# rehakvoj1/BIH-GPU-Raytracer

Hardware: NVIDIA B200
Metric: Mrays/s (higher is better)
Workload: dtype f32

## Files before the change

bih-gpu-raytracer_b200/csrc/trace.cu:

```cuda
#include "bihrt_internal.cuh"
#include <float.h>

#define FULL 0xffffffffu
#define NONE 0xFFFFFFFFu
#define TRACE_THREADS 128
#define TRACE_MIN_BLOCKS 8
constexpr int NODE_STEPS = 4;

#define OCT_MIXED 8
#define BOX_EPS 2.384185791015625e-07f

#define DET_EPS __uint_as_float(0x358637beu)

struct Hit { float t; int slot; };

__device__ __forceinline__ float fmin3(float a, float b, float c) { float r; asm("min.f32 %0, %1, %2, %3;" : "=f"(r) : "f"(a), "f"(b), "f"(c)); return r; }
__device__ __forceinline__ float fmax3(float a, float b, float c) { float r; asm("max.f32 %0, %1, %2, %3;" : "=f"(r) : "f"(a), "f"(b), "f"(c)); return r; }

__device__ __forceinline__ uint32_t pack_colour(uint32_t hits, int samples) {
    const float fh = (float)hits, fm = (float)(samples - (int)hits), fs = (float)samples;
    float cr = __fdiv_rn(__fadd_rn(__fmul_rn(fh, 255.f), __fmul_rn(fm, 20.f)), fs);
    float cb = __fdiv_rn(__fmul_rn(fm, 40.f), fs);
    cr = fmaxf(0.f, fminf(255.f, cr));
    cb = fmaxf(0.f, fminf(255.f, cb));
    return ((uint32_t)(int)cb << 16) | ((uint32_t)(int)cr << 8) | (uint32_t)(int)cr;
}

__device__ __forceinline__ float mt_det(float dx, float dy, float dz, float e1x, float e1y, float e1z, float e2x, float e2y, float e2z,
                                        float& px, float& py, float& pz) {
    px = __fsub_rn(__fmul_rn(dy, e2z), __fmul_rn(e2y, dz));
    py = __fsub_rn(__fmul_rn(dz, e2x), __fmul_rn(e2z, dx));
    pz = __fsub_rn(__fmul_rn(dx, e2y), __fmul_rn(e2x, dy));
    return __fadd_rn(__fadd_rn(__fmul_rn(e1x, px), __fmul_rn(e1y, py)), __fmul_rn(e1z, pz));
}
__device__ __forceinline__ float mt_u(float ox, float oy, float oz, const float4& q0, float px, float py, float pz, float inv,
                                      float& tx, float& ty, float& tz) {
    tx = __fsub_rn(ox, q0.x); ty = __fsub_rn(oy, q0.y); tz = __fsub_rn(oz, q0.z);
    return __fmul_rn(__fadd_rn(__fadd_rn(__fmul_rn(tx, px), __fmul_rn(ty, py)), __fmul_rn(tz, pz)), inv);
}
__device__ __forceinline__ float mt_v(float dx, float dy, float dz, float e1x, float e1y, float e1z, float tx, float ty, float tz, float inv,
                                      float& qx, float& qy, float& qz) {
    qx = __fsub_rn(__fmul_rn(ty, e1z), __fmul_rn(e1y, tz));
    qy = __fsub_rn(__fmul_rn(tz, e1x), __fmul_rn(e1z, tx));
    qz = __fsub_rn(__fmul_rn(tx, e1y), __fmul_rn(e1x, ty));
    return __fmul_rn(__fadd_rn(__fadd_rn(__fmul_rn(dx, qx), __fmul_rn(dy, qy)), __fmul_rn(dz, qz)), inv);
}

template <bool COUNTED, bool FIRST, bool RANGE = false, bool TWO_SIDED = false>
__device__ __forceinline__ void test_leaf(const char* __restrict__ first_tri, float ox, float oy, float oz,
                                          float dx, float dy, float dz, Hit& h, uint32_t& ntris, uint32_t& wleaf,
                                          const float* tlo_p = nullptr) {
    const float4* p = reinterpret_cast<const float4*>(first_tri);
    for (;;) {
        const float4 q0 = __ldg(p), q1 = __ldg(p + 1), q2 = __ldg(p + 2);
        if (COUNTED) { ntris++; const uint32_t am = __activemask(); wleaf += ((threadIdx.x & 31) == __ffs(am) - 1); }
        const float e1x = q0.w, e1y = q1.x, e1z = q1.y, e2x = q1.z, e2y = q1.w, e2z = q2.x;
        float px, py, pz;
        const float det = mt_det(dx, dy, dz, e1x, e1y, e1z, e2x, e2y, e2z, px, py, pz);
        if (!((TWO_SIDED ? fabsf(det) : det) < DET_EPS)) {
            const float inv = __frcp_rn(det);
            float tx, ty, tz;
            const float u = mt_u(ox, oy, oz, q0, px, py, pz, inv, tx, ty, tz);
            if (!(u < 0.f || u > 1.f)) {
                float qx, qy, qz;
                const float v = mt_v(dx, dy, dz, e1x, e1y, e1z, tx, ty, tz, inv, qx, qy, qz);
                if (!(v < 0.f || __fadd_rn(u, v) > 1.f)) {
                    const float t = __fmul_rn(__fadd_rn(__fadd_rn(__fmul_rn(e2x, qx), __fmul_rn(e2y, qy)), __fmul_rn(e2z, qz)), inv);
                    if (t > (RANGE ? *tlo_p : 0.f) && t < h.t) {
                        h.t = t; h.slot = (int)__float_as_uint(q2.w);
                        if (FIRST) break;
                    }
                }
            }
        }
        if (__float_as_uint(q2.z) & 1u) break;
        p += 3;
    }
}

template <int MODE, bool COUNTED, bool Q>
__global__ void __launch_bounds__(TRACE_THREADS, TRACE_MIN_BLOCKS) k_trace(TraceArgs a) {
    constexpr int STACK_DEPTH = Q ? STACK_DEPTH_QUALITY : STACK_DEPTH_PARITY;
    constexpr bool COVER = MODE == 1;
    constexpr bool OCTS = MODE == 1;
    constexpr bool LIST = MODE == 0 || MODE == 3 || MODE == 4;
    constexpr bool RANGE = MODE == 3 || MODE == 4;
    constexpr bool TWO_SIDED = MODE == 4;
    __shared__ __align__(16) float s_ray[TRACE_THREADS * 10];
    const int lane = threadIdx.x & 31;
    const uint32_t lt = (1u << lane) - 1u;
    float* my_ray = s_ray + threadIdx.x * 10;
    const char* __restrict__ nodes_b = reinterpret_cast<const char*>(a.nodes);
    const char* __restrict__ tris_b = reinterpret_cast<const char*>(a.tris);
    const BihTri* __restrict__ tris = a.tris;
    const uint32_t nu = a.hdr->nu;
    if (a.hdr->status != 0) return;
    if ((a.hdr->quality != 0) != Q) {
        if (blockIdx.x == 0 && threadIdx.x == 0 && a.status_map) *a.status_map = 0x100u;
        return;
    }
    const float blo[3] = { a.hdr->lo[0], a.hdr->lo[1], a.hdr->lo[2] }, bhi[3] = { a.hdr->hi[0], a.hdr->hi[1], a.hdr->hi[2] };
    uint32_t nnodes = 0, ntris = 0, maxsp = 0;
    uint32_t wnode = 0, wleaf = 0;

    uint64_t total;
    int tx = 1;
    if (LIST) total = a.tile_cost ? (((uint64_t)a.nrays + 1023u) >> 10) << 10 : (uint64_t)a.nrays;
    else {
        tx = (a.w + 31) / 32;
        const int ty = (a.h + 31) / 32, T = tx * ty;
        const int my_tiles = T > a.shard_index ? (T - a.shard_index + a.shard_count - 1) / a.shard_count : 0;
        total = ((uint64_t)my_tiles * 1024u) << a.gshift;
    }
    const int gshift = LIST ? 0 : a.gshift;
    const int nsamp = LIST ? 1 : ((a.s_end - a.s_begin) >> gshift);
    uint32_t my_queue = 0;
    if (a.queues > 1) { asm("mov.u32 %0, %%smid;" : "=r"(my_queue)); my_queue %= (uint32_t)a.queues; }
    uint64_t pool_next = 0, pool_end = 0;
    long long unit_t0 = 0; uint32_t unit_tile = 0xFFFFFFFFu;
    bool exhausted = false;

    uint64_t item = ~0ull;
    int s = 0, s0 = 0;
    uint32_t hits = 0, pixel = 0, pxy = 0;
    float ix = 1.f, iy = 1.f, iz = 1.f, nx = 0.f, ny = 0.f, nz = 0.f, bpad = 0.f;
    uint32_t cur = NONE;
    float rMin = 0.f, pMin = 0.f, pMax = 0.f;
    Hit h; h.t = FLT_MAX; h.slot = -1;
    bool tracing = false;
    uint4 stack[STACK_DEPTH];
    int sp = 0;
#define STACK_RESET() do { sp = 0; } while (0)
#define STACK_PUSH(item) do { stack[sp] = (item); sp++; } while (0)
#define STACK_POP(e) do { sp--; (e) = stack[sp]; } while (0)
    const uint32_t root_ref = BIH_REF_NODE(0, a.hdr->root_axis);
    const bool direct = MODE == 1 && gshift > 0 && !(a.flags & BIHRT_RENDER_COUNTS);
    const uint32_t ray_smem = (uint32_t)__cvta_generic_to_shared(my_ray);

    for (;;) {
        const uint32_t busy = ~__ballot_sync(FULL, cur == NONE);
        if (busy == 0) {
            bool want_item = false, finishing = false;
            if (cur == NONE) {
                if (tracing) {
                    tracing = false;
                    if (MODE == 1) hits += (h.slot >= 0);
                    else if (RANGE) {
                        const bool hit = h.slot >= 0;
                        const bool rec = a.out_u || a.out_v || a.out_ng;
                        float u = 0.f, v = 0.f, gx = 0.f, gy = 0.f, gz = 0.f;
                        int32_t prim = -1;
                        if (hit && (rec || a.out_prim)) {
                            const float4* tq = reinterpret_cast<const float4*>(tris + h.slot);
                            const float4 q0 = __ldg(tq), q1 = __ldg(tq + 1), q2 = __ldg(tq + 2);
                            prim = (int32_t)__float_as_uint(q2.y);
                            if (rec) {
                                const float e1x = q0.w, e1y = q1.x, e1z = q1.y, e2x = q1.z, e2y = q1.w, e2z = q2.x;
                                const float2 dxy = *reinterpret_cast<const float2*>(my_ray + 6);
                                const float dx = dxy.x, dy = dxy.y, dz = my_ray[8];
                                float px, py, pz, tx, ty, tz, qx, qy, qz;
                                const float inv = __frcp_rn(mt_det(dx, dy, dz, e1x, e1y, e1z, e2x, e2y, e2z, px, py, pz));
                                u = mt_u(my_ray[0], my_ray[2], my_ray[4], q0, px, py, pz, inv, tx, ty, tz);
                                v = mt_v(dx, dy, dz, e1x, e1y, e1z, tx, ty, tz, inv, qx, qy, qz);
                                gx = __fsub_rn(__fmul_rn(e1y, e2z), __fmul_rn(e1z, e2y));
                                gy = __fsub_rn(__fmul_rn(e1z, e2x), __fmul_rn(e1x, e2z));
                                gz = __fsub_rn(__fmul_rn(e1x, e2y), __fmul_rn(e1y, e2x));
                            }
                        }
                        if (a.out_t) a.out_t[item] = hit ? h.t : FLT_MAX;
                        if (a.out_slot) a.out_slot[item] = h.slot;
                        if (a.out_prim) a.out_prim[item] = prim;
                        if (a.out_u) a.out_u[item] = u;
                        if (a.out_v) a.out_v[item] = v;
                        if (a.out_ng) { float* g = a.out_ng + 3 * item; g[0] = gx; g[1] = gy; g[2] = gz; }
                    } else {
                        const uint64_t o = MODE == 0 ? item : (uint64_t)pixel * (uint32_t)a.spp + (uint32_t)(s0 + s);
                        if (a.out_t) a.out_t[o] = h.t;
                        if (a.out_slot) a.out_slot[o] = h.slot;
                        if (a.out_prim) a.out_prim[o] = h.slot >= 0 ? (int32_t)tris[h.slot].prim : -1;
                    }
                    s++;
                    if (s == nsamp) {
                        if (MODE == 1 && gshift > 0) finishing = true;
                        else if (MODE == 1 && (a.flags & BIHRT_RENDER_COUNTS)) a.fb[pixel] = hits;
                        else if (MODE == 1) a.fb[pixel] = pack_colour(hits, nsamp);
                        item = ~0ull;
                    }
                }
                want_item = (item == ~0ull);
            }
            if (MODE == 1 && gshift > 0) {
                const uint32_t fin = __ballot_sync(FULL, finishing);
                if (finishing) {
                    const uint32_t same = __match_any_sync(fin, pixel);
                    const uint32_t sum = __reduce_add_sync(same, hits);
                    if (lane == __ffs(same) - 1) {
                        if (direct) a.fb[pixel] = pack_colour(sum, nsamp << gshift);
                        else if (sum) atomicAdd(&a.fb[pixel], sum);
                    }
                }
            }
            if (!LIST && a.tile_cost && unit_tile != 0xFFFFFFFFu) {
                if (lane == 0) atomicMax(a.tile_cost + unit_tile, (uint32_t)min((unsigned long long)(clock64() - unit_t0) >> 8, 0xFFFFFFFFull));
                unit_tile = 0xFFFFFFFFu;
            }
            uint32_t want = __ballot_sync(FULL, want_item);
            while (want && !exhausted) {
                if (pool_next >= pool_end) {
                    uint64_t base = ~0ull;
                    uint32_t got = 0;
                    if (lane == 0) {
                        const uint32_t ilc = (uint32_t)a.il_count, ili = (uint32_t)a.il_index, ics = (uint32_t)a.il_cshift;
                        if (a.queues <= 1) {
                            const uint64_t fetched = atomicAdd(a.work, 32u); got = 32;
                            const uint64_t lu = fetched >> 5;
                            base = ilc > 1 ? ((((lu >> ics) * ilc + ili) << ics) | (lu & ((1u << ics) - 1u))) << 5 : fetched;
                            if (base >= total) base = ~0ull;
                        } else {
                            const uint32_t tshift = 10 + gshift, ushift = 5 + gshift;
                            const uint64_t ntile = (total + ((1ull << tshift) - 1)) >> tshift;
                            for (uint32_t k = 0; k < (uint32_t)a.queues; k++) {
                                uint32_t q = my_queue + k; if (q >= (uint32_t)a.queues) q -= (uint32_t)a.queues;
                                if (q >= ntile) continue;
                                const uint32_t upt = (1u << ushift) / ilc;
                                const uint64_t units = ((ntile - q + a.queues - 1) / a.queues) * upt;
                                if (ld_relaxed(a.work + q) >= units) continue;
                                const uint32_t u = atomicAdd(a.work + q, 1u);
                                if (u >= units) continue;
                                const uint32_t lu = u % upt;
                                const uint64_t b = (((uint64_t)(u / upt) * a.queues + q) << tshift) + ((uint64_t)((((lu >> ics) * ilc + ili) << ics) | (lu & ((1u << ics) - 1u))) << 5);
                                if (b < total) { base = b; got = 32; break; }
                            }
                        }
                    }
                    base = __shfl_sync(FULL, base, 0);
                    got = __shfl_sync(FULL, got, 0);
                    if (LIST && a.tile_cost && unit_tile != 0xFFFFFFFFu) {
                        if (lane == 0) atomicMax(a.tile_cost + unit_tile, (uint32_t)min((unsigned long long)(clock64() - unit_t0) >> 8, 0xFFFFFFFFull));
                        unit_tile = 0xFFFFFFFFu;
                    }
                    if (base == ~0ull) { exhausted = true; break; }
                    pool_next = base;
                    pool_end = min(base + got, total);
                    if (a.tile_cost && unit_tile == 0xFFFFFFFFu) {
                        const uint32_t m = (uint32_t)(base >> (10 + gshift));
                        unit_tile = a.tile_order ? __ldg(a.tile_order + m) : m;
                        unit_t0 = clock64();
                    }
                }
                const uint64_t avail = pool_end - pool_next;
                const uint32_t rank = __popc(want & lt);
                const bool served = want_item && (uint64_t)rank < avail;
                if (served) {
                    item = pool_next + rank; s = 0; hits = 0; want_item = false;
                    if (LIST && a.tile_cost) {
                        const uint32_t mi = (uint32_t)(item >> 10);
                        const uint64_t ray = ((uint64_t)(a.tile_order ? __ldg(a.tile_order + mi) : mi) << 10) | (item & 1023u);
                        item = ray < (uint64_t)a.nrays ? ray : ~0ull;
                        if (item == ~0ull) want_item = true;
                    }
                    if (MODE == 0 && a.perm && item != ~0ull) item = __ldg(a.perm + item);
                    if (!LIST) {
                        const uint64_t pix = item >> gshift;
                        s0 = a.s_begin + (int)((uint32_t)item & ((1u << gshift) - 1u)) * nsamp;
                        const uint32_t mi = (uint32_t)(pix >> 10), q = (uint32_t)pix & 1023u;
                        const uint32_t m = a.tile_order ? __ldg(a.tile_order + mi) : mi;
                        const int tile = a.shard_index + (int)m * a.shard_count;
                        const int px = (tile % tx) * 32 + (int)((q >> 5) & 3u) * 8 + (int)(q & 7u);
                        const int py = (tile / tx) * 32 + (int)(q >> 7) * 4 + (int)((q >> 3) & 3u);
                        if (px < a.w && py < a.h) { pixel = (uint32_t)(py * a.w + px); pxy = (uint32_t)px | ((uint32_t)py << 16); }
                        else item = ~0ull;
                        if (item == ~0ull) want_item = true;
                    }
                }
                pool_next += min((uint64_t)__popc(want), avail);
                want = __ballot_sync(FULL, want_item);
            }
            if (cur == NONE && item != ~0ull) {
                float ox, oy, oz, dx, dy, dz;
                float tlo = 0.f, thi = FLT_MAX;
                bool live = true;
                if (RANGE) {
                    const float4* p = reinterpret_cast<const float4*>(a.rays_iv + item);
                    const float4 r0 = __ldg(p), r1 = __ldg(p + 1);
                    ox = r0.x; oy = r0.y; oz = r0.z; dx = r1.x; dy = r1.y; dz = r1.z;
                    tlo = fmaxf(r0.w, 0.f);
                    live = r0.w == r0.w && tlo < r1.w;
                    thi = fminf(r1.w, FLT_MAX);
                } else if (MODE == 0) {
                    const float* p = reinterpret_cast<const float*>(a.rays + item);
                    ox = __ldg(p); oy = __ldg(p + 1); oz = __ldg(p + 2); dx = __ldg(p + 3); dy = __ldg(p + 4); dz = __ldg(p + 5);
                } else {
                    const int px = (int)(pxy & 0xFFFFu), py = (int)(pxy >> 16);
                    const float ru = (a.flags & BIHRT_RENDER_JITTER) ? bihrt_jitter(a.seed, pixel, (uint32_t)(s0 + s), 0) : 0.5f;
                    const float rv = (a.flags & BIHRT_RENDER_JITTER) ? bihrt_jitter(a.seed, pixel, (uint32_t)(s0 + s), 1) : 0.5f;
                    const float uu = __fdiv_rn(__fadd_rn((float)px, ru), (float)a.w);
                    const float vv = __fdiv_rn(__fadd_rn((float)py, rv), (float)a.h);
                    ox = a.cam.origin[0]; oy = a.cam.origin[1]; oz = a.cam.origin[2];
                    dx = __fsub_rn(__fadd_rn(__fadd_rn(a.cam.lower_left[0], __fmul_rn(uu, a.cam.horizontal[0])), __fmul_rn(vv, a.cam.vertical[0])), ox);
                    dy = __fsub_rn(__fadd_rn(__fadd_rn(a.cam.lower_left[1], __fmul_rn(uu, a.cam.horizontal[1])), __fmul_rn(vv, a.cam.vertical[1])), oy);
                    dz = __fsub_rn(__fadd_rn(__fadd_rn(a.cam.lower_left[2], __fmul_rn(uu, a.cam.horizontal[2])), __fmul_rn(vv, a.cam.vertical[2])), oz);
                }
                ix = __frcp_rn(dx); iy = __frcp_rn(dy); iz = __frcp_rn(dz);
                nx = -__fmul_rn(ox, ix); ny = -__fmul_rn(oy, iy); nz = -__fmul_rn(oz, iz);
                bpad = __fmul_rn(BOX_EPS, fmaxf(fmaxf(fabsf(nx) <= FLT_MAX ? fabsf(nx) : 0.f, fabsf(ny) <= FLT_MAX ? fabsf(ny) : 0.f),
                                                fabsf(nz) <= FLT_MAX ? fabsf(nz) : 0.f));
                *reinterpret_cast<float2*>(my_ray) = make_float2(ox, ix); *reinterpret_cast<float2*>(my_ray + 2) = make_float2(oy, iy);
                *reinterpret_cast<float2*>(my_ray + 4) = make_float2(oz, iz); *reinterpret_cast<float2*>(my_ray + 6) = make_float2(dx, dy);
                my_ray[8] = dz;
                if (RANGE) my_ray[9] = tlo;
                h.t = RANGE ? thi : (MODE == 0 && a.any_hit) ? a.tmax : FLT_MAX; h.slot = -1; STACK_RESET(); tracing = true;
                bool in = nu > 0 && live;
                float tMin = __fmul_rn(__fsub_rn(ix < 0.f ? bhi[0] : blo[0], ox), ix);
                float tMax = __fmul_rn(__fsub_rn(ix < 0.f ? blo[0] : bhi[0], ox), ix);
                const float tymin = __fmul_rn(__fsub_rn(iy < 0.f ? bhi[1] : blo[1], oy), iy);
                const float tymax = __fmul_rn(__fsub_rn(iy < 0.f ? blo[1] : bhi[1], oy), iy);
                if ((tMin > tymax) || (tymin > tMax)) in = false;
                if (tymin > tMin) tMin = tymin;
                if (tymax < tMax) tMax = tymax;
                const float tzmin = __fmul_rn(__fsub_rn(iz < 0.f ? bhi[2] : blo[2], oz), iz);
                const float tzmax = __fmul_rn(__fsub_rn(iz < 0.f ? blo[2] : bhi[2], oz), iz);
                if ((tMin > tzmax) || (tzmin > tMax)) in = false;
                if (tzmin > tMin) tMin = tzmin;
                if (tzmax < tMax) tMax = tzmax;
                if (in) {
                    const float tabs = fmaxf(fabsf(tMin), fabsf(tMax));
                    bpad = __fmaf_rn(BOX_EPS, tabs <= FLT_MAX ? tabs : FLT_MAX, bpad);
                    const float qnan = __uint_as_float(0x7fc00000u);
                    ix = fabsf(ix) <= FLT_MAX ? ix : qnan; iy = fabsf(iy) <= FLT_MAX ? iy : qnan; iz = fabsf(iz) <= FLT_MAX ? iz : qnan;
                    rMin = tMin; pMin = fmaxf(tMin, tlo); pMax = ((MODE == 0 && a.any_hit) || COVER || RANGE) ? fminf(tMax, h.t) : tMax;
                    if (nu == 1) { cur = BIH_REF_LEAFREF(0); pMin = -FLT_MAX; pMax = FLT_MAX; }
                    else if (pMin <= pMax) cur = root_ref;
                }
            }
            if (OCTS) {
                int oct = OCT_MIXED;
                if (gshift > 0) {
                    const bool w = cur != NONE;
                    const uint32_t xn = __ballot_sync(FULL, w && ix < 0.f), xp = __ballot_sync(FULL, w && ix > 0.f);
                    const uint32_t yn = __ballot_sync(FULL, w && iy < 0.f), yp = __ballot_sync(FULL, w && iy > 0.f);
                    const uint32_t zn = __ballot_sync(FULL, w && iz < 0.f), zp = __ballot_sync(FULL, w && iz > 0.f);
                    if (!((xn && xp) || (yn && yp) || (zn && zp))) oct = (xn != 0) | (yn != 0) << 1 | (zn != 0) << 2;
                }
                my_ray[9] = __int_as_float(oct);
            }
            if (__ballot_sync(FULL, cur != NONE || tracing) == 0 && exhausted &&
                __ballot_sync(FULL, item != ~0ull) == 0) break;
        }

#define BOX_SLAB(lx, ly, lz, hx, hy, hz, bn, bf)                                                            \
        do {                                                                                                \
            const float ax0 = __fmaf_rn((lx), ix, nx), ax1 = __fmaf_rn((hx), ix, nx);                       \
            const float ay0 = __fmaf_rn((ly), iy, ny), ay1 = __fmaf_rn((hy), iy, ny);                       \
            const float az0 = __fmaf_rn((lz), iz, nz), az1 = __fmaf_rn((hz), iz, nz);                       \
            float n_, f_;                                                                                   \
            if (OCT == OCT_MIXED) {                                                                         \
                n_ = fmaxf(fmaxf(fminf(ax0, ax1), fminf(ay0, ay1)), fminf(az0, az1));                       \
                f_ = fminf(fminf(fmaxf(ax0, ax1), fmaxf(ay0, ay1)), fmaxf(az0, az1));                       \
            } else {                                             \
                n_ = fmax3((OCT & 1) ? ax1 : ax0, (OCT & 2) ? ay1 : ay0, (OCT & 4) ? az1 : az0);            \
                f_ = fmin3((OCT & 1) ? ax0 : ax1, (OCT & 2) ? ay0 : ay1, (OCT & 4) ? az0 : az1);            \
            }                                                                                               \
            (bn) = __fsub_rn(n_, bpad);                                                                     \
            (bf) = __fadd_rn(f_, bpad);                                                                     \
        } while (0)
#define POP_VALID()                                                                                         \
        do {                                                                                                \
            cur = NONE;                                                                                     \
            if (COVER) {                                   \
                if (sp > 0) {                                                                               \
                    uint4 e;                                                                                \
                    STACK_POP(e);                                                                           \
                    cur = e.x; rMin = __uint_as_float(e.y); pMin = __uint_as_float(e.z); pMax = __uint_as_float(e.w); \
                }                                                                                           \
            } else while (sp > 0) {                                                                         \
                uint4 e;                                                                                    \
                STACK_POP(e);                                                                               \
                const float m = fminf(__uint_as_float(e.w), h.t);                                           \
                if (__uint_as_float(e.z) <= m) { cur = e.x; rMin = __uint_as_float(e.y); pMin = __uint_as_float(e.z); pMax = m; break; } \
            }                                                                                               \
        } while (0)
#ifdef BIHRT_DEBUG_STACK
#define DEBUG_STACK_TRAP() do { if (sp >= STACK_DEPTH) __trap(); } while (0)
#else
#define DEBUG_STACK_TRAP() do { } while (0)
#endif
#define NODE_PHASE(OCT_)                                                                                           \
        do {                                                                                                        \
            constexpr int OCT = (OCT_);                                                                             \
            for (;;) {                                                                                              \
                _Pragma("unroll (NODE_STEPS)")                                                                      \
                for (int rep = 0; rep < NODE_STEPS && (int)cur >= 0; rep++) {                                       \
                                    \
                    float2 oi;                                                                                      \
                    uint32_t ra;                                                                                    \
                    asm("mad.lo.u32 %0, %1, 8, %2;" : "=r"(ra) : "r"(cur & 3u), "r"(ray_smem));                     \
                    asm volatile("ld.shared.v2.f32 {%0, %1}, [%2];" : "=f"(oi.x), "=f"(oi.y) : "r"(ra));            \
                           \
                    const float4* np;                                                                               \
                    asm("mad.wide.u32 %0, %1, 64, %2;" : "=l"(np) : "r"(cur >> 2), "l"(nodes_b));                   \
                     \
                     \
                     \
                     \
                     \
                                                                          \
                    float4 nd, b0, b1, b2;                                                                          \
                    if (LIST) {                                                                                     \
                        asm("ld.global.nc.v8.f32 {%0,%1,%2,%3,%4,%5,%6,%7}, [%8];"                                  \
                            : "=f"(nd.x), "=f"(nd.y), "=f"(nd.z), "=f"(nd.w), "=f"(b0.x), "=f"(b0.y), "=f"(b0.z), "=f"(b0.w) : "l"(np)); \
                        asm("ld.global.nc.v8.f32 {%0,%1,%2,%3,%4,%5,%6,%7}, [%8];"                                  \
                            : "=f"(b1.x), "=f"(b1.y), "=f"(b1.z), "=f"(b1.w), "=f"(b2.x), "=f"(b2.y), "=f"(b2.z), "=f"(b2.w) : "l"(np + 2)); \
                    } else { nd = __ldg(np); b0 = __ldg(np + 1); b1 = __ldg(np + 2); b2 = __ldg(np + 3); }          \
                    if (COUNTED) { nnodes++; const uint32_t am = __activemask(); wnode += (lane == __ffs(am) - 1); } \
                    const uint32_t rl = __float_as_uint(nd.z), rr = __float_as_uint(nd.w);                          \
                    const bool neg = oi.y < 0.f;                                       \
                    const float t0 = __fmul_rn(__fsub_rn(nd.x, oi.x), oi.y);                          \
                    const float t1 = __fmul_rn(__fsub_rn(nd.y, oi.x), oi.y);                                        \
                    const float tn = neg ? t1 : t0, tf = neg ? t0 : t1;                                             \
                    const uint32_t refn = neg ? rr : rl, reff = neg ? rl : rr;                                      \
                     \
                     \
                     \
                     \
                                                              \
                    float bnL, bfL, bnR, bfR;                                                                       \
                    BOX_SLAB(b0.x, b0.y, b0.z, b0.w, b1.x, b1.y, bnL, bfL);                                         \
                    BOX_SLAB(b1.z, b1.w, b2.x, b2.y, b2.z, b2.w, bnR, bfR);                                         \
                     \
                    const float nLo = fmaxf(pMin, neg ? bnR : bnL), nHi = fmin3(pMax, tn, neg ? bfR : bfL);         \
                    const float fLo = fmax3(pMin, tf, neg ? bnL : bnR), fHi = fminf(pMax, neg ? bfL : bfR);         \
                    const bool go_near = (Q || rMin < tn) && (nLo <= nHi);    \
                    const bool go_far = (fLo <= fHi);                                                               \
                     \
                          \
                    if (go_near && go_far) {                                                                        \
                             \
                        if ((int)refn >= 0 && (int)reff < 0) {                                                      \
                            STACK_PUSH(make_uint4(refn, __float_as_uint(rMin), __float_as_uint(nLo), __float_as_uint(nHi))); \
                            cur = reff; rMin = tf; pMin = fLo; pMax = fHi;                                          \
                        } else {                                                                                    \
                            STACK_PUSH(make_uint4(reff, __float_as_uint(tf), __float_as_uint(fLo), __float_as_uint(fHi))); \
                            cur = refn; pMin = nLo; pMax = nHi;                                                     \
                        }                                                                                           \
                         \
                         \
                                                           \
                        if (COUNTED) { maxsp = max(maxsp, (uint32_t)sp); if (sp >= STACK_DEPTH) { maxsp = 0x7fffffffu; sp = STACK_DEPTH - 1; } } \
                        DEBUG_STACK_TRAP();                                                                         \
                    } else if (go_near) { cur = refn; pMin = nLo; pMax = nHi; }                                     \
                    else if (go_far) { cur = reff; rMin = tf; pMin = fLo; pMax = fHi; }                             \
                    else POP_VALID();                                                                               \
                }                                                                                                   \
                const uint32_t m_walk = __ballot_sync(FULL, (int)cur >= 0);                                         \
                if (m_walk == 0) break;                                                                             \
                const uint32_t m_wait = __ballot_sync(FULL, cur + 1u > 0x80000000u);   \
                if (__popc(m_wait) > __popc(m_walk)) break;                                                         \
            }                                                                                                       \
        } while (0)
        if constexpr (!OCTS) NODE_PHASE(OCT_MIXED);
        else switch (__float_as_int(my_ray[9])) {
            case 0: NODE_PHASE(0); break;
            case 1: NODE_PHASE(1); break;
            case 2: NODE_PHASE(2); break;
            case 3: NODE_PHASE(3); break;
            case 4: NODE_PHASE(4); break;
            case 5: NODE_PHASE(5); break;
            case 6: NODE_PHASE(6); break;
            case 7: NODE_PHASE(7); break;
            default: NODE_PHASE(OCT_MIXED); break;
        }
        if (cur + 1u > 0x80000000u) {
            const char* tp;
            asm("mad.wide.u32 %0, %1, 12, %2;" : "=l"(tp) : "r"(cur & 0x7FFFFFFCu), "l"(tris_b));
            const float2 dxy = *reinterpret_cast<const float2*>(my_ray + 6);
            test_leaf<COUNTED, COVER, RANGE, TWO_SIDED>(tp, my_ray[0], my_ray[2], my_ray[4], dxy.x, dxy.y, my_ray[8], h, ntris, wleaf, my_ray + 9);
            if (((LIST && a.any_hit) || COVER) && h.slot >= 0) { STACK_RESET(); cur = NONE; }
            else POP_VALID();
        }
#undef NODE_PHASE
#undef DEBUG_STACK_TRAP
#undef POP_VALID
#undef BOX_SLAB
#undef STACK_RESET
#undef STACK_PUSH
#undef STACK_POP
        __syncwarp();
    }

    if (COUNTED) {
#pragma unroll
        for (int o = 16; o > 0; o >>= 1) {
            nnodes += __shfl_xor_sync(FULL, nnodes, o);
            ntris += __shfl_xor_sync(FULL, ntris, o);
            maxsp = max(maxsp, __shfl_xor_sync(FULL, maxsp, o));
        }
        if (lane == 0) {
            atomicAdd(&a.counters[0], (unsigned long long)nnodes);
            atomicAdd(&a.counters[1], (unsigned long long)ntris);
            atomicMax(&a.counters[2], (unsigned long long)maxsp);
        }
        wnode = __reduce_add_sync(FULL, wnode); wleaf = __reduce_add_sync(FULL, wleaf);
        if (lane == 0) { atomicAdd(&a.counters[4], (unsigned long long)wnode); atomicAdd(&a.counters[5], (unsigned long long)wleaf); }
    }
}

__global__ void k_resolve(uint32_t* fb, int npix, int spp) {
    const int i = blockIdx.x * blockDim.x + threadIdx.x;
    if (i >= npix) return;
    fb[i] = pack_colour(fb[i], spp);
}

#define TILE_CLASSES 5
__device__ __forceinline__ int tile_class(uint32_t c, uint32_t mx) {
    int k = 0;
#pragma unroll
    for (int j = 1; j < TILE_CLASSES; j++) k += c < max(1u, mx >> j);
    return k;
}
__global__ void __launch_bounds__(1024) k_tile_order(uint32_t* __restrict__ cost, uint32_t* __restrict__ order, uint32_t ntiles) {
    __shared__ uint32_t s_w[TILE_CLASSES][32];
    __shared__ uint32_t s_max, s_base[TILE_CLASSES];
    const int lane = threadIdx.x & 31, w = threadIdx.x >> 5;
    const uint32_t per = (ntiles + 1023u) / 1024u, i0 = min(ntiles, threadIdx.x * per), i1 = min(ntiles, i0 + per);
    uint32_t mx = 0;
    for (uint32_t i = i0; i < i1; i++) mx = max(mx, cost[i]);
    mx = __reduce_max_sync(0xffffffffu, mx);
    if (lane == 0) s_w[0][w] = mx;
    __syncthreads();
    if (threadIdx.x == 0) { uint32_t m = 0; for (int k = 0; k < 32; k++) m = max(m, s_w[0][k]); s_max = m; }
    __syncthreads();
    mx = s_max;
    uint32_t cnt[TILE_CLASSES], inc[TILE_CLASSES];
#pragma unroll
    for (int k = 0; k < TILE_CLASSES; k++) cnt[k] = 0;
    for (uint32_t i = i0; i < i1; i++) {
        const int cl = tile_class(cost[i], mx);
#pragma unroll
        for (int k = 0; k < TILE_CLASSES; k++) cnt[k] += (cl == k);
    }
    __syncthreads();
#pragma unroll
    for (int k = 0; k < TILE_CLASSES; k++) {
        inc[k] = cnt[k];
#pragma unroll
        for (int o = 1; o < 32; o <<= 1) { const uint32_t t = __shfl_up_sync(0xffffffffu, inc[k], o); if (lane >= o) inc[k] += t; }
        if (lane == 31) s_w[k][w] = inc[k];
    }
    __syncthreads();
    if (threadIdx.x < TILE_CLASSES) {
        uint32_t run = 0;
        for (int j = 0; j < 32; j++) { const uint32_t x = s_w[threadIdx.x][j]; s_w[threadIdx.x][j] = run; run += x; }
        s_base[threadIdx.x] = run;
    }
    __syncthreads();
    if (threadIdx.x == 0) { uint32_t run = 0; for (int k = 0; k < TILE_CLASSES; k++) { const uint32_t x = s_base[k]; s_base[k] = run; run += x; } }
    __syncthreads();
    uint32_t pos[TILE_CLASSES];
#pragma unroll
    for (int k = 0; k < TILE_CLASSES; k++) pos[k] = s_base[k] + s_w[k][w] + inc[k] - cnt[k];
    for (uint32_t i = i0; i < i1; i++) {
        const int cl = tile_class(cost[i], mx);
#pragma unroll
        for (int k = 0; k < TILE_CLASSES; k++) if (cl == k) order[pos[k]++] = i;
    }
    __syncthreads();
    for (uint32_t i = i0; i < i1; i++) cost[i] = 0;
}

__global__ void __launch_bounds__(1024) k_tile_sort(uint32_t* __restrict__ cost, uint32_t* __restrict__ order, uint32_t ntiles) {
    __shared__ uint32_t s_cnt[256], s_off[256];
    if (threadIdx.x < 256) s_cnt[threadIdx.x] = 0;
    __syncthreads();
    for (uint32_t i = threadIdx.x; i < ntiles; i += 1024) atomicAdd(&s_cnt[min(255u, cost[i] >> 4)], 1u);
    __syncthreads();
    if (threadIdx.x == 0) { uint32_t run = 0; for (int b = 255; b >= 0; b--) { s_off[b] = run; run += s_cnt[b]; } }
    __syncthreads();
    for (uint32_t i = threadIdx.x; i < ntiles; i += 1024) order[atomicAdd(&s_off[min(255u, cost[i] >> 4)], 1u)] = i;
    __syncthreads();
    for (uint32_t i = threadIdx.x; i < ntiles; i += 1024) cost[i] = 0;
}

int bihrt_tile_order_launch(bihrt_ctx* c, uint32_t* cost, uint32_t* order, uint32_t ntiles, bool full_sort) {
    if (full_sort) k_tile_sort<<<1, 1024, 0, c->stream>>>(cost, order, ntiles);
    else k_tile_order<<<1, 1024, 0, c->stream>>>(cost, order, ntiles);
    c->kernel_launches += 1;
    BIHRT_CUDA(c, cudaGetLastError());
    return BIHRT_OK;
}

int bihrt_resolve_launch(bihrt_ctx* c, uint32_t* fb, int npix, int spp) {
    k_resolve<<<(npix + 255) / 256, 256, 0, c->stream>>>(fb, npix, spp);
    c->kernel_launches += 1;
    BIHRT_CUDA(c, cudaGetLastError());
    return BIHRT_OK;
}

template <int MODE, bool COUNTED, bool Q>
static int launch(bihrt_ctx* c, const TraceArgs& a) {
    int per_sm = c->opt_trace_blocks_per_sm;
    if (per_sm <= 0) {
        BIHRT_CUDA(c, cudaOccupancyMaxActiveBlocksPerMultiprocessor(&per_sm, k_trace<MODE, COUNTED, Q>, TRACE_THREADS, 0));
        if (per_sm < 1) per_sm = 1;
    }
    BIHRT_CUDA(c, cudaMemsetAsync(a.work, 0, 4 * 1024, c->stream));
    k_trace<MODE, COUNTED, Q><<<c->sm_count * per_sm, TRACE_THREADS, 0, c->stream>>>(a);
    c->kernel_launches += 1;
    BIHRT_CUDA(c, cudaGetLastError());
    return BIHRT_OK;
}

template <bool Q>
static int launch_mode(bihrt_ctx* c, const TraceArgs& a, int mode, bool counted) {
    switch (mode * 2 + (counted ? 1 : 0)) {
        case 0: return launch<0, false, Q>(c, a);
        case 1: return launch<0, true, Q>(c, a);
        case 2: return launch<1, false, Q>(c, a);
        case 3: return launch<1, true, Q>(c, a);
        case 4: return launch<2, false, Q>(c, a);
        case 5: return launch<2, true, Q>(c, a);
        case 6: return launch<3, false, Q>(c, a);
        case 8: return launch<4, false, Q>(c, a);
        default: return bihrt_fail(c, BIHRT_ERR_INVALID, "bad trace mode %d", mode);
    }
}

int bihrt_trace_launch(bihrt_ctx* c, const TraceArgs& a_in, int mode, bool counted) {
    TraceArgs a = a_in;
    const bool list = mode == 0 || mode == 3 || mode == 4;
    const int64_t rays = list ? a.nrays : (int64_t)a.w * a.h * (a.s_end - a.s_begin) / (a.shard_count > 0 ? a.shard_count : 1) / (a.il_count > 0 ? a.il_count : 1);
    const bool on = a.queues < 0 ? (rays >= (16ll << 20) && (list || a.gshift == 0)) : a.queues != 0;
    a.queues = on ? (c->sm_count < 1024 ? c->sm_count : 1024) : 1;
    uint32_t ntiles = 0;
    bihrt_ctx::TileKey key;
    if (!list) {
        const int tx = (a.w + 31) / 32, ty = (a.h + 31) / 32, T = tx * ty;
        const int mine = T > a.shard_index ? (T - a.shard_index + a.shard_count - 1) / a.shard_count : 0;
        if ((((uint64_t)mine * 1024u) << a.gshift) >= (1ull << 32) - (1ull << 24))
            return bihrt_fail(c, BIHRT_ERR_INVALID, "launch of %d tiles x 1024 pixels x %d lane groups exceeds the 32-bit work counter", mine, 1 << a.gshift);
    }
    const bool order_on = a.queues == 1 && (c->opt_tile_order > 1 || (c->opt_tile_order == 1 && rays >= (64ll << 10) && rays < (48ll << 20) && c->n >= 10000));
    if (order_on) {
        if (list) {
            if (a.nrays > 1024 && a.nrays <= (65536ll << 10)) { ntiles = (uint32_t)((a.nrays + 1023) >> 10); key.nrays = a.nrays; }
        } else {
            const int tx = (a.w + 31) / 32, ty = (a.h + 31) / 32, T = tx * ty;
            const int mine = T > a.shard_index ? (T - a.shard_index + a.shard_count - 1) / a.shard_count : 0;
            if (mine > 1 && mine <= 65536) ntiles = (uint32_t)mine;
            key.w = a.w; key.h = a.h; key.gshift = a.gshift; key.nsamp = a.s_end - a.s_begin; key.shard_index = a.shard_index;
            key.shard_count = a.shard_count; key.il_index = a.il_index; key.il_count = a.il_count; key.il_cshift = a.il_cshift;
        }
        key.mode = list ? mode : 1; key.ntiles = ntiles;
    }
    bihrt_ctx::TileSlot* slot = nullptr;
    if (ntiles) {
        for (auto& ts : c->tile_slots) if (ts.cap && ts.key == key) slot = &ts;
        if (!slot) {
            slot = &c->tile_slots[c->tile_next];
            c->tile_next = (c->tile_next + 1) % 4;
            slot->key = key; slot->valid = false;
        }
        if ((size_t)ntiles > slot->cap) {
            if (slot->cost) cudaFree(slot->cost);
            if (slot->order) cudaFree(slot->order);
            slot->cost = slot->order = nullptr; slot->cap = 0; slot->valid = false;
            if (cudaMalloc(&slot->cost, (size_t)ntiles * 4) != cudaSuccess || cudaMalloc(&slot->order, (size_t)ntiles * 4) != cudaSuccess) {
                cudaGetLastError();
                if (slot->cost) { cudaFree(slot->cost); slot->cost = nullptr; }
                slot = nullptr; ntiles = 0;
            } else slot->cap = ntiles;
        }
        if (slot) {
            if (!slot->valid) BIHRT_CUDA(c, cudaMemsetAsync(slot->cost, 0, (size_t)ntiles * 4, c->stream));
            a.tile_cost = slot->cost;
            a.tile_order = slot->valid ? slot->order : nullptr;
        }
    }
    a.status_map = c->d_status_map;
    int rc = c->built_quality ? launch_mode<true>(c, a, mode, counted) : launch_mode<false>(c, a, mode, counted);
    if (rc == BIHRT_OK && slot) {
        if ((rc = bihrt_tile_order_launch(c, slot->cost, slot->order, ntiles, rays < c->opt_tile_sort_below)) == BIHRT_OK) slot->valid = true;
    }
    return rc;
}
```

Baseline: 14690.

## Pack ray slab math into f32x2 ops and spill per-lane state to shared memory

Rewrites the box-slab and split-plane tests to use paired f32x2 FMA/add/mul instructions on packed 64-bit ray constants. Moves rarely used per-lane scalars (pixel, pxy, s0, unit timestamp) into shared memory, narrows the work-pool counters to 32-bit, and loads the scene bounds only at ray setup. The aim is fewer FP instructions and lower register pressure in the traversal loop, which may allow better occupancy. The costs are extra pack/unpack moves and shared-memory traffic for the moved state, and 32-bit counters that overflow if the work total is very large.

```diff
diff --git a/bih-gpu-raytracer_b200/csrc/trace.cu b/bih-gpu-raytracer_b200/csrc/trace.cu
--- a/bih-gpu-raytracer_b200/csrc/trace.cu
+++ b/bih-gpu-raytracer_b200/csrc/trace.cu
@@ -16,6 +16,18 @@
 
 __device__ __forceinline__ float fmin3(float a, float b, float c) { float r; asm("min.f32 %0, %1, %2, %3;" : "=f"(r) : "f"(a), "f"(b), "f"(c)); return r; }
 __device__ __forceinline__ float fmax3(float a, float b, float c) { float r; asm("max.f32 %0, %1, %2, %3;" : "=f"(r) : "f"(a), "f"(b), "f"(c)); return r; }
+
+__device__ __forceinline__ uint64_t f2_hold(float x, float y) { uint64_t r; asm volatile("mov.b64 %0, {%1, %2};" : "=l"(r) : "f"(x), "f"(y)); return r; }
+__device__ __forceinline__ float f2_x(uint64_t p) { float x, y; asm("mov.b64 {%0, %1}, %2;" : "=f"(x), "=f"(y) : "l"(p)); return x; }
+__device__ __forceinline__ float f2_y(uint64_t p) { float x, y; asm("mov.b64 {%0, %1}, %2;" : "=f"(x), "=f"(y) : "l"(p)); return y; }
+__device__ __forceinline__ float2 f2_fma(float2 a, uint64_t b, uint64_t c) {
+    uint64_t r; asm("{ .reg .b64 t; mov.b64 t, {%1, %2}; fma.rn.f32x2 %0, t, %3, %4; }" : "=l"(r) : "f"(a.x), "f"(a.y), "l"(b), "l"(c));
+    return make_float2(f2_x(r), f2_y(r));
+}
+__device__ __forceinline__ float2 f2_add(float2 a, uint64_t b) {
+    uint64_t r; asm("{ .reg .b64 t; mov.b64 t, {%1, %2}; add.rn.f32x2 %0, t, %3; }" : "=l"(r) : "f"(a.x), "f"(a.y), "l"(b));
+    return make_float2(f2_x(r), f2_y(r));
+}
 
 __device__ __forceinline__ uint32_t pack_colour(uint32_t hits, int samples) {
     const float fh = (float)hits, fm = (float)(samples - (int)hits), fs = (float)samples;
@@ -99,31 +111,36 @@
         if (blockIdx.x == 0 && threadIdx.x == 0 && a.status_map) *a.status_map = 0x100u;
         return;
     }
-    const float blo[3] = { a.hdr->lo[0], a.hdr->lo[1], a.hdr->lo[2] }, bhi[3] = { a.hdr->hi[0], a.hdr->hi[1], a.hdr->hi[2] };
     uint32_t nnodes = 0, ntris = 0, maxsp = 0;
     uint32_t wnode = 0, wleaf = 0;
 
-    uint64_t total;
+    uint32_t total;
     int tx = 1;
-    if (LIST) total = a.tile_cost ? (((uint64_t)a.nrays + 1023u) >> 10) << 10 : (uint64_t)a.nrays;
+    if (LIST) total = (uint32_t)(a.tile_cost ? (((uint64_t)a.nrays + 1023u) >> 10) << 10 : (uint64_t)a.nrays);
     else {
         tx = (a.w + 31) / 32;
         const int ty = (a.h + 31) / 32, T = tx * ty;
         const int my_tiles = T > a.shard_index ? (T - a.shard_index + a.shard_count - 1) / a.shard_count : 0;
-        total = ((uint64_t)my_tiles * 1024u) << a.gshift;
+        total = (uint32_t)(((uint64_t)my_tiles * 1024u) << a.gshift);
     }
     const int gshift = LIST ? 0 : a.gshift;
     const int nsamp = LIST ? 1 : ((a.s_end - a.s_begin) >> gshift);
     uint32_t my_queue = 0;
     if (a.queues > 1) { asm("mov.u32 %0, %%smid;" : "=r"(my_queue)); my_queue %= (uint32_t)a.queues; }
-    uint64_t pool_next = 0, pool_end = 0;
-    long long unit_t0 = 0; uint32_t unit_tile = 0xFFFFFFFFu;
+    uint32_t pool_next = 0, pool_end = 0;
+    uint32_t unit_tile = 0xFFFFFFFFu;
+    __shared__ long long s_unit_t0[TRACE_THREADS / 32];
+    long long& unit_t0 = s_unit_t0[threadIdx.x >> 5];
     bool exhausted = false;
 
     uint64_t item = ~0ull;
-    int s = 0, s0 = 0;
-    uint32_t hits = 0, pixel = 0, pxy = 0;
-    float ix = 1.f, iy = 1.f, iz = 1.f, nx = 0.f, ny = 0.f, nz = 0.f, bpad = 0.f;
+    int s = 0;
+    uint32_t hits = 0;
+    __shared__ uint32_t s_lane[3][TRACE_THREADS];
+    int& s0 = *reinterpret_cast<int*>(&s_lane[0][threadIdx.x]);
+    uint32_t& pixel = s_lane[1][threadIdx.x]; uint32_t& pxy = s_lane[2][threadIdx.x];
+    s0 = 0; pixel = 0; pxy = 0;
+    uint64_t i_xy = f2_hold(1.f, 1.f), i_zx = i_xy, n_xy = f2_hold(0.f, 0.f), n_zx = n_xy, pad = n_xy;
     uint32_t cur = NONE;
     float rMin = 0.f, pMin = 0.f, pMax = 0.f;
     Hit h; h.t = FLT_MAX; h.slot = -1;
@@ -200,8 +217,8 @@
                     }
                 }
             }
-            if (!LIST && a.tile_cost && unit_tile != 0xFFFFFFFFu) {
-                if (lane == 0) atomicMax(a.tile_cost + unit_tile, (uint32_t)min((unsigned long long)(clock64() - unit_t0) >> 8, 0xFFFFFFFFull));
+            if (!LIST && a.tile_cost && lane == 0 && unit_tile != 0xFFFFFFFFu) {
+                atomicMax(a.tile_cost + unit_tile, (uint32_t)min((unsigned long long)(clock64() - unit_t0) >> 8, 0xFFFFFFFFull));
                 unit_tile = 0xFFFFFFFFu;
             }
             uint32_t want = __ballot_sync(FULL, want_item);
@@ -233,24 +250,24 @@
                             }
                         }
                     }
-                    base = __shfl_sync(FULL, base, 0);
+                    const uint32_t first = __shfl_sync(FULL, (uint32_t)base, 0);
                     got = __shfl_sync(FULL, got, 0);
-                    if (LIST && a.tile_cost && unit_tile != 0xFFFFFFFFu) {
-                        if (lane == 0) atomicMax(a.tile_cost + unit_tile, (uint32_t)min((unsigned long long)(clock64() - unit_t0) >> 8, 0xFFFFFFFFull));
+                    if (LIST && a.tile_cost && lane == 0 && unit_tile != 0xFFFFFFFFu) {
+                        atomicMax(a.tile_cost + unit_tile, (uint32_t)min((unsigned long long)(clock64() - unit_t0) >> 8, 0xFFFFFFFFull));
                         unit_tile = 0xFFFFFFFFu;
                     }
-                    if (base == ~0ull) { exhausted = true; break; }
-                    pool_next = base;
-                    pool_end = min(base + got, total);
-                    if (a.tile_cost && unit_tile == 0xFFFFFFFFu) {
-                        const uint32_t m = (uint32_t)(base >> (10 + gshift));
+                    if (first == ~0u) { exhausted = true; break; }
+                    pool_next = first;
+                    pool_end = min(first + got, total);
+                    if (a.tile_cost && lane == 0 && unit_tile == 0xFFFFFFFFu) {
+                        const uint32_t m = first >> (10 + gshift);
                         unit_tile = a.tile_order ? __ldg(a.tile_order + m) : m;
                         unit_t0 = clock64();
                     }
                 }
-                const uint64_t avail = pool_end - pool_next;
+                const uint32_t avail = pool_end - pool_next;
                 const uint32_t rank = __popc(want & lt);
-                const bool served = want_item && (uint64_t)rank < avail;
+                const bool served = want_item && rank < avail;
                 if (served) {
                     item = pool_next + rank; s = 0; hits = 0; want_item = false;
                     if (LIST && a.tile_cost) {
@@ -273,7 +290,7 @@
                         if (item == ~0ull) want_item = true;
                     }
                 }
-                pool_next += min((uint64_t)__popc(want), avail);
+                pool_next += min((uint32_t)__popc(want), avail);
                 want = __ballot_sync(FULL, want_item);
             }
             if (cur == NONE && item != ~0ull) {
@@ -301,15 +318,16 @@
                     dy = __fsub_rn(__fadd_rn(__fadd_rn(a.cam.lower_left[1], __fmul_rn(uu, a.cam.horizontal[1])), __fmul_rn(vv, a.cam.vertical[1])), oy);
                     dz = __fsub_rn(__fadd_rn(__fadd_rn(a.cam.lower_left[2], __fmul_rn(uu, a.cam.horizontal[2])), __fmul_rn(vv, a.cam.vertical[2])), oz);
                 }
-                ix = __frcp_rn(dx); iy = __frcp_rn(dy); iz = __frcp_rn(dz);
-                nx = -__fmul_rn(ox, ix); ny = -__fmul_rn(oy, iy); nz = -__fmul_rn(oz, iz);
-                bpad = __fmul_rn(BOX_EPS, fmaxf(fmaxf(fabsf(nx) <= FLT_MAX ? fabsf(nx) : 0.f, fabsf(ny) <= FLT_MAX ? fabsf(ny) : 0.f),
+                float ix = __frcp_rn(dx), iy = __frcp_rn(dy), iz = __frcp_rn(dz);
+                const float nx = -__fmul_rn(ox, ix), ny = -__fmul_rn(oy, iy), nz = -__fmul_rn(oz, iz);
+                float bpad = __fmul_rn(BOX_EPS, fmaxf(fmaxf(fabsf(nx) <= FLT_MAX ? fabsf(nx) : 0.f, fabsf(ny) <= FLT_MAX ? fabsf(ny) : 0.f),
                                                 fabsf(nz) <= FLT_MAX ? fabsf(nz) : 0.f));
                 *reinterpret_cast<float2*>(my_ray) = make_float2(ox, ix); *reinterpret_cast<float2*>(my_ray + 2) = make_float2(oy, iy);
                 *reinterpret_cast<float2*>(my_ray + 4) = make_float2(oz, iz); *reinterpret_cast<float2*>(my_ray + 6) = make_float2(dx, dy);
                 my_ray[8] = dz;
                 if (RANGE) my_ray[9] = tlo;
                 h.t = RANGE ? thi : (MODE == 0 && a.any_hit) ? a.tmax : FLT_MAX; h.slot = -1; STACK_RESET(); tracing = true;
+                const float blo[3] = { a.hdr->lo[0], a.hdr->lo[1], a.hdr->lo[2] }, bhi[3] = { a.hdr->hi[0], a.hdr->hi[1], a.hdr->hi[2] };
                 bool in = nu > 0 && live;
                 float tMin = __fmul_rn(__fsub_rn(ix < 0.f ? bhi[0] : blo[0], ox), ix);
                 float tMax = __fmul_rn(__fsub_rn(ix < 0.f ? blo[0] : bhi[0], ox), ix);
@@ -332,11 +350,14 @@
                     if (nu == 1) { cur = BIH_REF_LEAFREF(0); pMin = -FLT_MAX; pMax = FLT_MAX; }
                     else if (pMin <= pMax) cur = root_ref;
                 }
+                i_xy = f2_hold(ix, iy); i_zx = f2_hold(iz, ix); n_xy = f2_hold(nx, ny); n_zx = f2_hold(nz, nx);
+                pad = f2_hold(-bpad, bpad);
             }
             if (OCTS) {
                 int oct = OCT_MIXED;
                 if (gshift > 0) {
                     const bool w = cur != NONE;
+                    const float ix = f2_x(i_xy), iy = f2_y(i_xy), iz = f2_x(i_zx);
                     const uint32_t xn = __ballot_sync(FULL, w && ix < 0.f), xp = __ballot_sync(FULL, w && ix > 0.f);
                     const uint32_t yn = __ballot_sync(FULL, w && iy < 0.f), yp = __ballot_sync(FULL, w && iy > 0.f);
                     const uint32_t zn = __ballot_sync(FULL, w && iz < 0.f), zp = __ballot_sync(FULL, w && iz > 0.f);
@@ -348,11 +369,11 @@
                 __ballot_sync(FULL, item != ~0ull) == 0) break;
         }
 
-#define BOX_SLAB(lx, ly, lz, hx, hy, hz, bn, bf)                                                            \
+#define BOX_SLAB(p0, p1, p2, bn, bf)                                                                        \
         do {                                                                                                \
-            const float ax0 = __fmaf_rn((lx), ix, nx), ax1 = __fmaf_rn((hx), ix, nx);                       \
-            const float ay0 = __fmaf_rn((ly), iy, ny), ay1 = __fmaf_rn((hy), iy, ny);                       \
-            const float az0 = __fmaf_rn((lz), iz, nz), az1 = __fmaf_rn((hz), iz, nz);                       \
+            const float2 d0 = f2_fma((p0), i_xy, n_xy), d1 = f2_fma((p1), i_zx, n_zx);                      \
+            const float ax0 = d0.x, ay0 = d0.y, az0 = d1.x, ax1 = d1.y;                                     \
+            const float ay1 = __fmaf_rn((p2).x, f2_y(i_xy), f2_y(n_xy)), az1 = __fmaf_rn((p2).y, f2_x(i_zx), f2_x(n_zx)); \
             float n_, f_;                                                                                   \
             if (OCT == OCT_MIXED) {                                                                         \
                 n_ = fmaxf(fmaxf(fminf(ax0, ax1), fminf(ay0, ay1)), fminf(az0, az1));                       \
@@ -361,8 +382,8 @@
                 n_ = fmax3((OCT & 1) ? ax1 : ax0, (OCT & 2) ? ay1 : ay0, (OCT & 4) ? az1 : az0);            \
                 f_ = fmin3((OCT & 1) ? ax0 : ax1, (OCT & 2) ? ay0 : ay1, (OCT & 4) ? az0 : az1);            \
             }                                                                                               \
-            (bn) = __fsub_rn(n_, bpad);                                                                     \
-            (bf) = __fadd_rn(f_, bpad);                                                                     \
+            const float2 nf_ = f2_add(make_float2(n_, f_), pad);                                            \
+            (bn) = nf_.x; (bf) = nf_.y;                                                                     \
         } while (0)
 #define POP_VALID()                                                                                         \
         do {                                                                                                \
@@ -415,8 +436,9 @@
                     if (COUNTED) { nnodes++; const uint32_t am = __activemask(); wnode += (lane == __ffs(am) - 1); } \
                     const uint32_t rl = __float_as_uint(nd.z), rr = __float_as_uint(nd.w);                          \
                     const bool neg = oi.y < 0.f;                                       \
-                    const float t0 = __fmul_rn(__fsub_rn(nd.x, oi.x), oi.y);                          \
-                    const float t1 = __fmul_rn(__fsub_rn(nd.y, oi.x), oi.y);                                        \
+                     \
+                    const float2 t01 = __fmul2_rn(__fadd2_rn(make_float2(nd.x, nd.y), make_float2(-oi.x, -oi.x)), make_float2(oi.y, oi.y)); \
+                    const float t0 = t01.x, t1 = t01.y;                                                             \
                     const float tn = neg ? t1 : t0, tf = neg ? t0 : t1;                                             \
                     const uint32_t refn = neg ? rr : rl, reff = neg ? rl : rr;                                      \
                      \
@@ -425,8 +447,8 @@
                      \
                                                               \
                     float bnL, bfL, bnR, bfR;                                                                       \
-                    BOX_SLAB(b0.x, b0.y, b0.z, b0.w, b1.x, b1.y, bnL, bfL);                                         \
-                    BOX_SLAB(b1.z, b1.w, b2.x, b2.y, b2.z, b2.w, bnR, bfR);                                         \
+                    BOX_SLAB(make_float2(b0.x, b0.y), make_float2(b0.z, b0.w), make_float2(b1.x, b1.y), bnL, bfL); \
+                    BOX_SLAB(make_float2(b1.z, b1.w), make_float2(b2.x, b2.y), make_float2(b2.z, b2.w), bnR, bfR); \
                      \
                     const float nLo = fmaxf(pMin, neg ? bnR : bnL), nHi = fmin3(pMax, tn, neg ? bfR : bfL);         \
                     const float fLo = fmax3(pMin, tf, neg ? bnL : bnR), fHi = fminf(pMax, neg ? bfL : bfR);         \
```

Result: faster. 15250, median of 6 (+3.8%).
